# HengWeiBin/CenterFusionDetect3D

Hardware: AMD Instinct MI355X
Metric: frames/sec/GPU CenterFusion forward, 3x448x800 bs=16; 1/2/4/8-GPU scaling (higher is better)
Workload: dtype f32 storage + f32 accumulate; products as split-operand MFMA passes: f16x3 backbone/neck (3 passes), heads' first 3x3 layers fp16 main term + block-scaled FP6 e2m3 cross terms (1.5 passes), heads' 1x1 layers bf16x3; 1 GPU; Centerfusion_Middle (DLA-34 + DCNv2 neck + pc_dep frustum fusion, 7+4 heads) forward + NMS/top-100 decode + 2D->3D postProcess, bs=16/GPU, 3x448x800, 50-200 radar pts/frame, random-init weights; global_batch=16, parallelism=dp1 (batch shard, async all-gather of the final boxes)

## Files before the change

centerfusiondetect3d_amd/_lib.py:

```python
import ctypes as C
import os

_PKG = os.path.dirname(os.path.abspath(__file__))
LIB_PATH = os.path.join(_PKG, "libcfhip.so")

ABI_VERSION = 7
CF_MAX_SRC = 4
CF_MAX_GROUPS = 4
ACT_NONE, ACT_RELU, ACT_SIGMOID_CLAMP, ACT_RAW_AND_SIGDEPTH = 0, 1, 2, 3
LAYOUT_NHWC, LAYOUT_NCHW = 0, 1

_f = C.c_void_p


class ConvArgs(C.Structure):
    _fields_ = [("src", _f * CF_MAX_SRC), ("src_c", C.c_int32 * CF_MAX_SRC), ("n_src", C.c_int32),
                ("B", C.c_int32), ("H", C.c_int32), ("W", C.c_int32), ("Ho", C.c_int32),
                ("Wo", C.c_int32), ("stride", C.c_int32), ("weight", _f), ("slots", _f),
                ("bias", _f), ("K_pad", C.c_int32), ("N", C.c_int32), ("N_pad", C.c_int32),
                ("residual", _f), ("res_stride", C.c_int32), ("out", _f), ("out2", _f),
                ("out_stride", C.c_int32), ("out_layout", C.c_int32), ("act", C.c_int32),
                ("precise", C.c_int32), ("out_scale", C.c_float), ("in_scale", C.c_float)]


# ... 106 lines not shown
class HeadTrainArgs(C.Structure):
    _fields_ = [("x", _f), ("x2", _f), ("x_stride", C.c_int32), ("c_x", C.c_int32), ("x2_stride", C.c_int32),
                ("c_x2", C.c_int32), ("B", C.c_int32), ("h", C.c_int32), ("w", C.c_int32), ("n_hidden", C.c_int32),
                ("hidden", C.c_int32), ("n_out", C.c_int32), ("chunk_px", C.c_int32),
                ("weight", _f * _HT_LAYERS), ("bias", _f * _HT_LAYERS), ("y", _f), ("gy", _f),
                ("gw", _f * _HT_LAYERS), ("gb", _f * _HT_LAYERS), ("workspace", _f), ("workspace_bytes", C.c_size_t)]


CF_TARGETS_MAX_OBJS = 128
CF_TARGETS_F = 20
TGT_HAS_AMODAL, TGT_HAS_ATTRIBUTES, TGT_HAS_VELOCITY, TGT_HAS_ALPHA = 1, 2, 4, 8
TGT_HAS_DEPTH, TGT_HAS_DIMENSION, TGT_HAS_LOCATION, TGT_HAS_YAW = 16, 32, 64, 128
TGT_REP3D, TGT_NORM2D, TGT_WRITE_DEPTH, TGT_WRITE_ROT, TGT_FRUSTUM = 1, 2, 4, 8, 16


class TargetsArgs(C.Structure):
    _fields_ = [("ann", _f), ("iann", _f), ("counts", _f), ("trans", _f), ("calib", _f), ("scale", _f), ("pc_dep", _f),
                ("B", C.c_int32), ("M", C.c_int32), ("C", C.c_int32), ("h", C.c_int32), ("w", C.c_int32),
                ("flags", C.c_int32), ("max_pc_dist", C.c_float),
                ("heat", _f), ("cls", _f), ("mask", _f), ("trunc_mask", _f), ("wh", _f), ("reg", _f), ("amodal_offset", _f),
                ("dimension", _f), ("depth", _f), ("rotbin", _f), ("rotres", _f), ("att", _f), ("att_mask", _f),
                ("velocity", _f), ("pc_hm", _f), ("t_bboxes", _f), ("t_scores", _f), ("t_centers", _f),
                ("t_heat_centers", _f), ("t_bboxes3d", _f), ("t_rotation", _f), ("t_att", _f), ("t_velocity", _f),
                ("workspace", _f), ("workspace_bytes", C.c_size_t)]


_i, _d = C.c_int, C.c_double
SYMBOLS = {
    "cf_conv2d_fused": (_i, [C.POINTER(ConvArgs), _f]),
    "cf_conv2d_f16x3": (_i, [C.POINTER(ConvArgs), _f]),
    "cf_conv3x3_f16x3": (_i, [C.POINTER(ConvArgs), _f]),
    "cf_conv3x3_root_f16x3": (_i, [C.POINTER(ConvArgs), C.POINTER(ConvArgs), C.POINTER(C.c_int32), _f]),
    "cf_conv3x3_proj_f16x3": (_i, [C.POINTER(ConvArgs), C.POINTER(C.c_int32), _f]),
    "cf_conv3x3_f16x3_grouped": (_i, [C.POINTER(C.POINTER(ConvArgs)), C.c_int32, _f]),
    "cf_conv3x3_grouped_form": (_i, [C.POINTER(C.POINTER(ConvArgs)), C.c_int32, C.POINTER(C.c_int32)]),
    "cf_conv3x3_tile_form": (_i, [C.c_int32, C.POINTER(C.POINTER(ConvArgs)), C.c_int32, C.POINTER(C.c_int32), C.POINTER(C.c_int32)]),
    "cf_stem_fused": (_i, [C.POINTER(StemArgs), _f]),
    "cf_stem_fused_early": (_i, [C.POINTER(StemEarlyArgs), _f]),
    "cf_split_bf16": (_i, [_f, _f, C.c_long, _i, _i, _i, _f]),
    "cf_head_fused": (_i, [C.POINTER(HeadFusedArgs), _f]),
    "cf_head_fused_with": (_i, [C.POINTER(HeadFusedArgs), _i, _i, _f]),
    "cf_head_fused_at": (_i, [C.POINTER(HeadFusedArgs), _f, _i, _f]),
    "cf_head_slot_tables": (_i, [_f, _f, _i, _i, _i, _f, _f, _f]),
    "cf_pack_feat_mx": (_i, [_f, _i, _f, C.c_long, _f]),
    "cf_pack_feat_mx_scaled": (_i, [_f, _i, _f, C.c_long, C.c_float, _f]),
    "cf_absmax_f32": (_i, [_f, C.c_long, _i, _i, _f, _f]),
    "cf_dcn_v2_fused": (_i, [C.POINTER(DcnArgs), _f]),
    "cf_dcn_v2_f16x3": (_i, [C.POINTER(DcnArgs), _f]),
    "cf_dcn_v2_workspace_bytes": (C.c_size_t, [_i, _i, _i, _i, _i]),
    "cf_dcn_v2_f16x3_grouped": (_i, [C.POINTER(C.POINTER(DcnArgs)), C.c_int32, _f]),
    "cf_dcn_v2_f16x3_form": (_i, [C.POINTER(C.POINTER(DcnArgs)), C.c_int32, C.POINTER(C.c_int32)]),
    "cf_gemm_tile_form": (_i, [C.c_long, _i, _i, _i, _i, _i, _i, C.POINTER(C.c_int32), C.POINTER(C.c_int32), C.POINTER(C.c_int32)]),
    "cf_dcn_v2_bwd_data": (_i, [C.POINTER(DcnBwdArgs), _f]),
    "cf_dcn_v2_bwd_weight": (_i, [C.POINTER(DcnBwdArgs), _f]),
    "cf_dcn_v2_bwd_workspace_bytes": (C.c_size_t, [_i, _i, _i, _i, _i]),
    "cf_loss_forward": (_i, [C.POINTER(LossArgs), _f]),
    "cf_loss_backward": (_i, [C.POINTER(LossArgs), _f]),
    "cf_loss_workspace_bytes": (C.c_size_t, [_i, _i, _i, _i]),
    "cf_targets_build": (_i, [C.POINTER(TargetsArgs), _f]),
    "cf_targets_workspace_bytes": (C.c_size_t, [_i, _i]),
    "cf_head_train_forward": (_i, [C.POINTER(HeadTrainArgs), _f]),
    "cf_head_backward": (_i, [C.POINTER(HeadTrainArgs), _f]),
    "cf_head_train_workspace_bytes": (C.c_size_t, [_i, _i, _i, _i, _i, _i]),
    "cf_head_bwd_workspace_bytes": (C.c_size_t, [_i, _i, _i, _i, _i, _i]),
    "cf_head_bwd_chunk_px": (_i, [_i, _i, _i, _i]),
    "cf_head_backward_dx": (_i, [C.POINTER(HeadTrainArgs), _f, _i, _f, _i, _f]),
# ... 96 lines not shown
```

centerfusiondetect3d_amd/build.py:

```python
import glob
import os
import shutil
import subprocess
import sys

PKG = os.path.dirname(os.path.abspath(__file__))
ROOT = os.path.dirname(PKG)
CSRC = os.path.join(PKG, "csrc")
OBJ = os.path.join(PKG, "_build")
LIB = os.path.join(PKG, "libcfhip.so")

ARCH = "gfx950"
COMMON = os.environ.get("CF_EXTRA_FLAGS", "").split() + ["-O3", "-std=c++17", "-fPIC", f"-I{os.path.join(ROOT, 'include')}", f"-I{CSRC}"]
SOURCES = [
    ("cf_gemm.hip", []),
    ("cf_gemm_f16.hip", []),
    ("cf_dcn_bwd.hip", []),
    ("cf_neck_bwd.hip", []),
    ("cf_base_bwd.hip", []),
    ("cf_conv3x3_f16.hip", []),
    ("cf_stem.hip", []),
    ("cf_stem_early.hip", []),
    ("cf_heads.hip", []),
    ("cf_heads_bwd.hip", []),
    ("cf_elementwise.hip", []),
    ("cf_topk.hip", ["-ffp-contract=off"]),
    ("cf_frustum.hip", ["-ffp-contract=off"]),
    ("cf_decode.hip", ["-ffp-contract=off"]),
    ("cf_radar.hip", ["-ffp-contract=off"]),
    ("cf_augment.hip", ["-ffp-contract=off"]),
    ("cf_loss.hip", []),
    ("cf_targets.hip", ["-ffp-contract=off"]),
    ("cf_pack.cpp", ["-ffp-contract=off"]),
    ("cf_error.cpp", []),
]


def sources_sha():
    import hashlib
    h = hashlib.sha256()
    files = sorted(glob.glob(os.path.join(CSRC, "*")) + glob.glob(os.path.join(ROOT, "include", "*.h")))
    for f in files:
        h.update(os.path.relpath(f, ROOT).encode() + b"\0")
        h.update(open(f, "rb").read())
    return h.hexdigest()


def _hipcc():
    exe = shutil.which("hipcc") or "/opt/rocm/bin/hipcc"
    if not os.path.exists(exe):
        raise RuntimeError("hipcc not found: cannot build libcfhip.so")
    return exe

# ... 33 lines not shown
```

centerfusiondetect3d_amd/model.py:

```python
import math
import threading
from typing import List

import torch
from torch import nn

from . import _lib, ops, packing
from .packing import Source
from .plan import AT_TIMED, SECONDARY_HEADS, _Plan, feat_operand
from .streams import (_CAPTURE_LOCK, _PROBE_LOG, _PROBE_US, _SIDE_STREAMS,
                      _concurrent, _pick_streams, _side_streams)

CHANNELS = [16, 32, 64, 128, 256, 512]


class _Scope(nn.Module):
    """Empty container: only exists so parameters get the reference's dotted names."""


def _register(root: nn.Module, dotted: str, tensor: torch.Tensor, buffer=False):
    mod = root
    parts = dotted.split(".")
    for p in parts[:-1]:
        if not hasattr(mod, p):
# ... 131 lines not shown
        self.fusionStrategy = config.MODEL.FUSION_STRATEGY if self.isRadarEnabled else None
        if self.fusionStrategy not in (None, "middle", "early"):
            raise NotImplementedError(f"fusion strategy {self.fusionStrategy!r} is outside the hot path")
        self.isEarly = early
        self.isFrustumEnabled = self.isRadarEnabled and bool(config.MODEL.FRUSTUM) and not early
        try:
            config.defrost()
            config.MODEL.PYRAMID_OUT_SIZE = [config.MODEL.OUTPUT_SIZE]
            config.freeze()
        except Exception:
            pass
        for name, tensor, is_buf in _param_spec(config):
            _register(self, name, tensor, is_buf)
        self._packed = None
        self._plans = {}
        self._plan_sets = {}
        self._graphs = {}
        self.max_plan_sets = 4
        self._lock = threading.RLock()
        self.precise = True
        self.conv_f16 = True
        self.lanes = True
        self.lanes_max_frames = 10
        self.streams = 2
        self.trunk_on_caller = True
        self.min_sub_batch = 6
        self.use_graph = False
        self.stem_fused = True
        self.stem_pool = True
        self.conv_patch = True
        self.neck_groups = True
        self.root_fuse = True
        self.root_fuse_children = False
        self.heads_lanes = True
        self.heads_at_peaks = True
        self.peaks_behind_frustum = True
        self.frustum_fused = True
        self.proj_fuse = True
        self.heads_bf16 = True
        self.heads_mx = True
        self._mx_active = False
        self.pack_mx_fused = True
        self.record_spans = False
        self.trunk_spans = []
        self._ranges = None
        self._feat_scale = ops.DEFAULT_IN_SCALE
        self.range_headroom = 8.0
        self._range_checked = False
        self.register_load_state_dict_post_hook(lambda m, _k: m._weights_changed())
        self.freezeBackbone = bool(getattr(config.MODEL, "FREEZE_BACKBONE", False))
        if self.freezeBackbone:
            for name, p in self.named_parameters():
                p.requires_grad_(name.startswith("detectHead_0."))
        self._stale = False
        self._neck_train = False
        self._base_train = False
        self.eval()

    def train(self, mode=True):
        super().train(mode)
        if not mode:
            self._repack_if_stale()
        return self

    def _repack_if_stale(self):
        if getattr(self, "_stale", False):
# ... 869 lines not shown
```

centerfusiondetect3d_amd/ops.py:

```python
import ctypes as C
from typing import Optional, Sequence

import torch

from . import _lib
from ._lib import (ACT_NONE, ACT_RELU, ACT_SIGMOID_CLAMP, ACT_RAW_AND_SIGDEPTH, LAYOUT_NHWC, LAYOUT_NCHW)
from .packing import PackedConv, PackedDcn, MX_ROW as packing_MX_ROW


def _need_cuda(*ts):
    for t in ts:
        if t is not None and not t.is_cuda:
            raise _lib.CfHipError("libcfhip operators need device tensors (no CPU path)")


DEFAULT_IN_SCALE = 16.0
F16_MAX = 65504.0


IN_SCALE_KEEP_MIN = 2.0 ** -6
IN_SCALE_MAX = 2.0 ** 32
F32_MIN_NORMAL = 2.0 ** -126


# ... 152 lines not shown
                       in_scale=None if in_scales is None else in_scales[g])
              for g, (p_, x) in enumerate(zip(pds, xs))]
    _lib.check(_lib.load().cf_dcn_v2_f16x3_grouped(group_ptrs(blocks), G, _lib.stream_ptr()), "cf_dcn_v2_f16x3_grouped")
    return out


def conv3x3_proj_f16x3(pc: PackedConv, t, pooled, act=ACT_RELU, out=None, in_scale=None):
    _need_cuda(t, pooled)
    assert pc.proj_k > 0, "weights packed without a projection"
    B, H, W, _ = t.shape
    if out is None:
        out = torch.empty((B, H, W, pc.n), device=t.device, dtype=torch.float32)
    a = conv_args(pc, [t, pooled], [t.shape[-1], pooled.shape[-1]], B, H, W, out, out.shape[-1], act, None, 0,
                  LAYOUT_NHWC, None, 0, False, in_scale=in_scale)
    ch = (C.c_int32 * 2)(*[int(c) for c in pc.real_cin])
    _lib.check(_lib.load().cf_conv3x3_proj_f16x3(C.byref(a), ch, _lib.stream_ptr()), "cf_conv3x3_proj_f16x3")
    return out


def conv3x3_root_f16x3(pc2: PackedConv, pc_root: PackedConv, t, x1, children=(), act_root=ACT_RELU, x2_out=None,
                       in_scale=None, root_in_scale=None):
    _need_cuda(t, x1, *children)
    B, H, W, _ = t.shape
    x2 = torch.empty((B, H, W, pc2.n), device=t.device, dtype=torch.float32) if x2_out is None else x2_out
    out = torch.empty((B, H, W, pc_root.n), device=t.device, dtype=torch.float32)
    a = conv_args(pc2, [t], [t.shape[-1]], B, H, W, x2, x2.shape[-1], ACT_RELU, x1, x1.shape[-1], LAYOUT_NHWC, None, 0, False,
                  in_scale=in_scale)
    srcs = [x2, x1, *children]
    r = conv_args(pc_root, srcs, [s.shape[-1] for s in srcs], B, H, W, out, out.shape[-1], act_root, None, 0,
                  LAYOUT_NHWC, None, 0, False, in_scale=root_in_scale)
    ch = (C.c_int32 * len(srcs))(*[int(c) for c in pc_root.real_cin])
    _lib.check(_lib.load().cf_conv3x3_root_f16x3(C.byref(a), C.byref(r), ch, _lib.stream_ptr()), "cf_conv3x3_root_f16x3")
    return out, x2


def run_conv(a: _lib.ConvArgs):
    _lib.check(_lib.load().cf_conv2d_fused(C.byref(a), _lib.stream_ptr()), "cf_conv2d_fused")


def conv2d_fused(pc: PackedConv, srcs, B, H, W, act=ACT_NONE, residual=None, layout=LAYOUT_NHWC,
                 out=None, out2=None, precise=True):
    _need_cuda(*srcs, residual)
    Ho = (H + 2 * pc.pad - pc.kh) // pc.stride + 1
    Wo = (W + 2 * pc.pad - pc.kh) // pc.stride + 1
    dev = srcs[0].device
    if out is None:
        shape = (B, Ho, Wo, pc.n) if layout == LAYOUT_NHWC else (B, pc.n, Ho, Wo)
        out = torch.empty(shape, device=dev, dtype=torch.float32)
    if act == ACT_RAW_AND_SIGDEPTH and out2 is None:
        out2 = torch.empty_like(out)
    a = conv_args(pc, srcs, [s.shape[-1] for s in srcs], B, H, W, out, pc.n, act, residual,
                  residual.shape[-1] if residual is not None else 0, layout, out2, 0, precise)
    run_conv(a)
    return (out, out2) if act == ACT_RAW_AND_SIGDEPTH else out


def split_bf16(x, channels=None, cs=None, out=None):
    _need_cuda(x)
    B, H, W, S = x.shape
    Cc = channels or S
    Cs = cs or ((Cc + 7) // 8) * 8
    if out is None:
        out = torch.empty((B, H, W, 2, Cs), device=x.device, dtype=torch.bfloat16)
    _lib.check(_lib.load().cf_split_bf16(x.data_ptr(), out.data_ptr(), B * H * W, Cc, S, Cs,
                                         _lib.stream_ptr()), "cf_split_bf16")
    return out
# ... 1426 lines not shown
```

centerfusiondetect3d_amd/plan.py:

```python
import ctypes as C
import weakref
from typing import Dict, List

import torch

from . import _lib, ops, packing
from .pending import PendingOutputs
from ._lib import (ACT_NONE, ACT_RELU, ACT_SIGMOID_CLAMP, ACT_RAW_AND_SIGDEPTH, LAYOUT_NHWC, LAYOUT_NCHW)
from .streams import _side_streams

SECONDARY_HEADS = ["velocity", "nuscenes_att", "depth2", "rotation2"]
AT_SLOTS = 18
AT_TIMED = ("at.topk", "at.peaks", "at.tables", "at.primary")


def feat_operand(model):
    if not model._heads_bf():
        return None
    return ((packing.MX_ROW,), torch.uint8) if model._mx_active else ((2, 64), torch.bfloat16)


def act_of(h):
    return ACT_SIGMOID_CLAMP if h == "heatmap" else (ACT_RAW_AND_SIGDEPTH if h in ("depth", "depth2") else ACT_NONE)


class _Plan:

    def __init__(self, model: "DLASeg", B, H, W, device, part="all", feat=None, feat_in=None):
        self.B, self.H, self.W, self.device = B, H, W, device
        self.h4, self.w4 = H // 4, W // 4
        self.part = part
        self.lib = _lib.load()
        self.steps = []
        self.lanes = []
        self.lane = 0
        self.n_events = 0
        self.use_lanes = bool(model.lanes) and part != "heads" and \
            B * (H // 4) * (W // 4) <= (model.lanes_max_frames if part == "all" else min(4, model.lanes_max_frames)) * 112 * 200
        self._side = self._events = None
        self.keep = []
        self.bytes = 0
        self.step_index = {}
        self.step_flops = {}
        self.timed = {}
        self.inputs = {}
        self.hidden = set()
        self.debug = {}
        self.in_step = self.stem = self.x4 = self.feat_producer = None
        self.early, self.direct_step, self.chained, self.feat_bf = bool(model.isEarly), None, [], None
        self._pooled = {}
        self._pre = {}
        self.primary, self.radar, self.frustum, self.K = [], False, False, int(model.config.MODEL.K)
# ... 2 lines not shown
        self.peaks_step = self.topk_step = self.frustum_step = None
        self.pc_hm4 = self.pc_hm8 = None
        self.tk_scores = self.tk_inds = self.tk_cls = self.tk_ws = None
        self.pk_ws = self.ev_peaks = None
        self.at, self.at_tails, self.group_flops, self.group_srcs, self._last = None, {}, {}, {}, None
        self.feat, self.feat_in = feat, feat_in
        self._m, self._pk = model, model._packed
        try:
            if part != "heads":
                self._build_trunk()
            if part not in ("trunk", "base", "stem"):
                self._build_heads()
        finally:
            self._m = self._pk = None

    def _buf(self, *shape, dtype=torch.float32):
        t = torch.empty(shape, device=self.device, dtype=dtype)
        self.bytes += t.numel() * t.element_size()
        self.keep.append(t)
        return t

    def _add(self, name, flops, step, *keep):
        self.keep += keep
        self.step_index[name] = len(self.steps)
        if flops is not None:
            self.step_flops[name] = flops
        self.add_step(step)
        return len(self.steps) - 1

    def _slot(self):
        self.add_step(None)
        return len(self.steps) - 1

    def _conv(self, name, srcs, h, w, act=ACT_RELU, residual=None, out=None, out_stride=None):
        m, B, pc = self._m, self.B, self._pk[name]
        ho = (h + 2 * pc.pad - pc.kh) // pc.stride + 1
        wo = (w + 2 * pc.pad - pc.kh) // pc.stride + 1
        if out is None:
            out = self._buf(B, ho, wo, pc.n)
        a = ops.conv_args(pc, srcs, [s.shape[-1] for s in srcs], B, h, w, out, out_stride or pc.n, act, residual,
                          residual.shape[-1] if residual is not None else 0, LAYOUT_NHWC, None, 0, m.precise,
                          in_scale=m._scale(name) if pc.out_scale > 0 else None)
        self.inputs[name] = list(srcs)
        fn = self.lib.cf_conv2d_fused
        if pc.out_scale > 0:
            fn = self.lib.cf_conv3x3_f16x3 if (pc.patch and m.conv_patch) else self.lib.cf_conv2d_f16x3
        self._add(name, 2.0 * B * ho * wo * pc.n * (pc.kh * pc.kh * sum(int(c) for c in pc.real_cin)), (fn, C.byref(a)), a)
        return out

    def _pool(self, x):
        if x.data_ptr() in self._pooled:
            return self._pooled[x.data_ptr()]
        _, h, w, c = x.shape
        o = self._buf(self.B, h // 2, w // 2, c)
        self.add_step((self.lib.cf_maxpool2x2, x.data_ptr(), o.data_ptr(), self.B, h, w, c))
        self._pooled[x.data_ptr()] = o
        return o

    def _block(self, p, x, residual, pooled=None):
        m, B = self._m, self.B
        _, h, w, _ = x.shape
        t = self._conv(p + ".conv1", [x], h, w)
        _, ho, wo, _ = t.shape
        if pooled is None:
            return self._conv(p + ".conv2", [t], ho, wo, residual=residual if residual is not None else x)
        pc = self._pk[p + ".conv2"]
        o = self._buf(B, ho, wo, pc.n)
        a = ops.conv_args(pc, [t, pooled], [t.shape[-1], pooled.shape[-1]], B, ho, wo, o, pc.n, ACT_RELU, None, 0,
                          LAYOUT_NHWC, None, 0, False, in_scale=m._scale(p + ".conv2"))
        self.inputs[p + ".conv2"], self.inputs[p[:-len(".tree1")] + ".project"] = [t], [pooled]
        ch = (C.c_int32 * 2)(*[int(c) for c in pc.real_cin])
        step = (self.lib.cf_conv3x3_proj_f16x3, C.byref(a), ch) if m.conv_patch else (self.lib.cf_conv2d_f16x3, C.byref(a))
        self._add(p + ".conv2+project", 2.0 * B * ho * wo * pc.n * (9 * pc.real_cin[0] + pc.real_cin[1]), step, a, ch)
        return o

    def _tree(self, p, levels, x, stride, level_root, children=None):
        m, B, pk = self._m, self.B, self._pk
        children = [] if children is None else children
        bottom = self._pool(x) if stride > 1 else x
        proj_fused = levels == 1 and getattr(pk[p + ".tree1.conv2"], "proj_k", 0) > 0
        if proj_fused:
            residual = None
        elif (p + ".project") in pk:
            _, h, w, _ = bottom.shape
            residual = self._conv(p + ".project", [bottom], h, w, act=ACT_NONE)
        else:
            residual = bottom
        if level_root:
            children.append(bottom)
        if levels > 1:
            x1 = self._tree(p + ".tree1", levels - 1, x, stride, False)
            children.append(x1)
            return self._tree(p + ".tree2", levels - 1, x1, 1, False, children)
        x1 = self._block(p + ".tree1", x, residual, pooled=bottom if proj_fused else None)
        _, h, w, _ = x1.shape
        pc2, pcr = pk[p + ".tree2.conv2"], pk[p + ".root"]
        if not (m.root_fuse and m.conv_patch and pc2.out_scale > 0 and pcr.out_scale > 0
                and getattr(pc2, "patch", False) and pc2.stride == 1 and (not children or m.root_fuse_children)):
            x2 = self._block(p + ".tree2", x1, None)
            return self._conv(p + ".root", [x2, x1, *children], h, w)
        t = self._conv(p + ".tree2.conv1", [x1], h, w)
        x2, o = self._buf(B, h, w, pc2.n), self._buf(B, h, w, pcr.n)
        a2 = ops.conv_args(pc2, [t], [t.shape[-1]], B, h, w, x2, pc2.n, ACT_RELU, x1, x1.shape[-1],
                           LAYOUT_NHWC, None, 0, False, in_scale=m._scale(p + ".tree2.conv2"))
        rsrcs = [x2, x1, *children]
        ar = ops.conv_args(pcr, rsrcs, [s_.shape[-1] for s_ in rsrcs], B, h, w, o, pcr.n, ACT_RELU, None, 0,
                           LAYOUT_NHWC, None, 0, False, in_scale=m._scale(p + ".root"))
        self.inputs[p + ".tree2.conv2"], self.inputs[p + ".root"] = [t], [x1, *children]
        self.hidden.add(p + ".root")
        rch = (C.c_int32 * len(rsrcs))(*[int(c) for c in pcr.real_cin])
        flops = 2.0 * B * h * w * (pc2.n * 9 * sum(int(c) for c in pc2.real_cin) + pcr.n * sum(int(c) for c in pcr.real_cin))
        self._add(p + ".tree2.conv2+root", flops, (self.lib.cf_conv3x3_root_f16x3, C.byref(a2), C.byref(ar), rch), a2, ar, rch)
        return o

    def _dcn_node(self, p, x, out=None, feat_producer=False):
        m, B = self._m, self.B
        _, h, w, c = x.shape
        om = self._buf(B, h, w, 32)
        self._conv(p + ".conv_offset_mask", [x], h, w, act=ACT_NONE, out=om, out_stride=32)
        pd = self._pk[p]
        o = self._buf(B, h, w, pd.n) if out is None else out
        ws = None
        if pd.out_scale > 0:
            nbytes = self.lib.cf_dcn_v2_workspace_bytes(B, h, w, pd.c, pd.n_pad)
            ws = self._buf(nbytes, dtype=torch.uint8) if nbytes else None
        a = ops.dcn_args(pd, x, om, 32, B, h, w, o, pd.n, ACT_RELU, precise=m.precise, workspace=ws,
                         in_scale=m._scale(p) if pd.out_scale > 0 else None)
        if feat_producer:
            self.feat_producer = a
        self.inputs[p] = [x]
        fn = self.lib.cf_dcn_v2_f16x3 if pd.out_scale > 0 else self.lib.cf_dcn_v2_fused
        self._add(p, 2.0 * B * h * w * pd.n * 9 * pd.c, (fn, C.byref(a)), a)
        return o
# ... 69 lines not shown
                           layers[i - 1].data_ptr(), summed.data_ptr(), self.B, h, w, c, f))
            layers[i] = self._dcn_node(f"{p}.node_{j}", summed, out=final_out if i == endp - 1 else None,
                                       feat_producer=feat and i == endp - 1)

    def _build_trunk(self):
        m, B, H, W, pk = self._m, self.B, self.H, self.W, self._pk
        if self.early and self.part == "all":
            self.direct_step = self._add("pc_hm_direct", 0.0, None)
        if "base.stem" in pk:
            y0, y1 = None, self._buf(B, H // 2, W // 2, 32)
            y1p = self._buf(B, H // 4, W // 4, 32) if m.stem_pool and self.part != "stem" else None
            if y1p is not None:
                self._pooled[y1.data_ptr()] = y1p
            stem_layers = ("base.base_layer", "base.level0", "base.level1")
            kw = dict(shape=(B, 3, H, W), out_pool=y1p, in_scales=[m._scale(n) for n in stem_layers])
            self.stem = ops.stem_early_args(pk["base.stem"], None, None, y1, **kw) if self.early else \
                ops.stem_args(pk["base.stem"], None, y1, **kw)
            self.hidden.update(stem_layers)
            k_base = 16 * 49 * (6 if self.early else 3)
            self.in_step = self._add("base.stem", 2.0 * B * H * W * (k_base + 16 * 144 + 32 * 144 / 4), None, self.stem)
        else:
            self.in_step = self._slot()
            self.x4 = self._buf(B, H, W, 8 if self.early else 4)
            if self.early:
                self.x4.zero_()
            t = self._conv("base.base_layer", [self.x4], H, W)
            y0 = self._conv("base.level0", [t], H, W)
            y1 = self._conv("base.level1", [y0], H, W)
        layers = [y0, y1]
        if self.part == "stem":
            self.levels = [y1]
            return
        for lvl, levels, root in ((2, 1, False), (3, 2, True), (4, 2, True), (5, 1, True)):
            layers.append(self._tree(f"base.level{lvl}", levels, layers[-1], 2, root))
        self.debug = {f"y{i}": t for i, t in enumerate(layers) if t is not None}
        if self.part == "base":
            self.levels = layers[2:]
            return
        out = [layers[-1]]
        n_ida = len(layers) - 2 - 1
        for i in range(n_ida):
            also = [("ida_up.proj_1", layers[-1])] if i == n_ida - 1 and i > 0 else []
            self._ida(f"dla_up.ida_{i}", layers, len(layers) - i - 2, len(layers), also=also)
            out.insert(0, layers[-1])
        for i, t in enumerate(out):
            self.debug[f"up{i}"] = t
        y = out[:3]
        self._ida("ida_up", y, 0, 3, final_out=self.feat, feat=True)
        feat = self.feat = y[-1]
        spec, pr, M4 = feat_operand(m), self.feat_producer, B * self.h4 * self.w4
        if spec is None:
            self.feat_in = feat
            return
        if self.feat_in is None:
            self.feat_in = self._buf(B, self.h4, self.w4, *spec[0], dtype=spec[1])
        if m._mx_active:
            if pr.out_scale > 0 and pr.N == 64 and pr.N_pad == 64 and bool(m.pack_mx_fused):
                pr.out_mx = self.feat_in.data_ptr()
                pr.mx_scale = m._feat_scale
                pr.workspace = None
            else:
                self._add("feat.pack_mx", None, (self.lib.cf_pack_feat_mx_scaled, feat.data_ptr(), 64, self.feat_in.data_ptr(),
                                                 C.c_long(M4), C.c_float(m._feat_scale)))
        elif pr.out_scale > 0 and pr.N == 64:
            pr.out_split_bf16, pr.split_stride = self.feat_in.data_ptr(), 64
            pr.workspace = None
        else:
# ... 387 lines not shown
```

include/cf_hip.h:

```cpp
#ifndef CF_HIP_H
#define CF_HIP_H

#include <stddef.h>
#include <stdint.h>

#ifdef __cplusplus
extern "C" {
#endif

#define CF_ABI_VERSION 7

#define CF_OK 0
#define CF_EINVAL (-22)
#define CF_ELAUNCH (-5)

#define CF_MAX_SRC 4
#define CF_MAX_GROUPS 4

#define CF_ACT_NONE 0
#define CF_ACT_RELU 1
#define CF_ACT_SIGMOID_CLAMP 2
#define CF_ACT_RAW_AND_SIGDEPTH 3

#define CF_LAYOUT_NHWC 0
// ... 29 lines not shown
  int32_t precise;
  float out_scale;
  float in_scale;
} cf_conv_args;
int cf_conv2d_fused(const cf_conv_args* a, void* stream);

typedef struct cf_stem_args {
  const float* x;
  int32_t B, C, H, W;
  const void* w_base;   const float* b_base;   float scale_base;
  const void* w_level0; const float* b_level0; float scale_level0;
  const void* w_level1; const float* b_level1; float scale_level1;
  float* out;
  float* out_pool;
  float in_scale[3];
} cf_stem_args;
int cf_stem_fused(const cf_stem_args* a, void* stream);

typedef struct cf_stem_early_args {
  cf_stem_args stem;
  const float* pc;
  int32_t pc_h, pc_w;
  const void* w_base_radar;
} cf_stem_early_args;
int cf_stem_fused_early(const cf_stem_early_args* a, void* stream);

int cf_conv2d_f16x3(const cf_conv_args* a, void* stream);

int cf_conv3x3_f16x3(const cf_conv_args* a, void* stream);

int cf_conv3x3_root_f16x3(const cf_conv_args* conv, const cf_conv_args* root, const int32_t* root_channels, void* stream);

int cf_conv3x3_proj_f16x3(const cf_conv_args* a, const int32_t* src_channels, void* stream);

int cf_conv3x3_f16x3_grouped(const cf_conv_args* const* groups, int32_t n_groups, void* stream);
int cf_conv3x3_grouped_form(const cf_conv_args* const* groups, int32_t n_groups, int32_t* form);

#define CF_CONV3_ENTRY_PLAIN 0
#define CF_CONV3_ENTRY_ROOT 1
#define CF_CONV3_ENTRY_PROJ 2
#define CF_CONV3_ENTRY_GROUPED 3
#define CF_CONV3_FORM_INTS 23
int cf_conv3x3_tile_form(int32_t entry, const cf_conv_args* const* blocks, int32_t n_blocks, const int32_t* channels, int32_t* form);

typedef struct cf_pack_src {
  int32_t channels;
  int32_t stride;
  int32_t c_base;
} cf_pack_src;
typedef struct cf_pack_bn {
  const float* gamma; const float* beta; const float* mean; const float* var;
  float eps;
} cf_pack_bn;
typedef struct cf_pack_conv_desc {
  const float* weight;
  const float* bias;
  cf_pack_bn bn;
  int32_t cout, kh, kw, stride;
  int32_t pad;
  int32_t dilation;
  const cf_pack_src* src; int32_t n_src;
  const float* proj_weight;
  const float* proj_bias;
  cf_pack_bn proj_bn;
  cf_pack_src proj;
} cf_pack_conv_desc;
// ... 394 lines not shown
```

Measured before the change: 3186 frames/s.

## Add specialised f16x3 GEMM kernel for DLA tree root 1x1 convolutions

Adds a dedicated kernel for the 1x1 root convolutions of the DLA trees. It reads the concatenated multi-source input directly, splits it into hi/lo fp16 in double-buffered LDS, keeps a register ring of weight fragments, and writes bias and ReLU through an LDS-staged epilogue. It is meant to replace the generic f16x3 conv path, with a tile form picked so the grid fits in one round. An optional fused 2x2 max-pool output is also added but is off by default; in exchange the change brings more kernel instantiations and a new dispatch heuristic.

```diff
diff --git a/centerfusiondetect3d_amd/_lib.py b/centerfusiondetect3d_amd/_lib.py
--- a/centerfusiondetect3d_amd/_lib.py
+++ b/centerfusiondetect3d_amd/_lib.py
@@ -162,6 +162,8 @@
     "cf_conv3x3_f16x3": (_i, [C.POINTER(ConvArgs), _f]),
     "cf_conv3x3_root_f16x3": (_i, [C.POINTER(ConvArgs), C.POINTER(ConvArgs), C.POINTER(C.c_int32), _f]),
     "cf_conv3x3_proj_f16x3": (_i, [C.POINTER(ConvArgs), C.POINTER(C.c_int32), _f]),
+    "cf_root1x1_f16x3": (_i, [C.POINTER(ConvArgs), C.POINTER(C.c_int32), _f, _f]),
+    "cf_root1x1_f16x3_form": (_i, [C.POINTER(ConvArgs), C.POINTER(C.c_int32), C.c_int32, C.POINTER(C.c_int32)]),
     "cf_conv3x3_f16x3_grouped": (_i, [C.POINTER(C.POINTER(ConvArgs)), C.c_int32, _f]),
     "cf_conv3x3_grouped_form": (_i, [C.POINTER(C.POINTER(ConvArgs)), C.c_int32, C.POINTER(C.c_int32)]),
     "cf_conv3x3_tile_form": (_i, [C.c_int32, C.POINTER(C.POINTER(ConvArgs)), C.c_int32, C.POINTER(C.c_int32), C.POINTER(C.c_int32)]),
diff --git a/centerfusiondetect3d_amd/build.py b/centerfusiondetect3d_amd/build.py
--- a/centerfusiondetect3d_amd/build.py
+++ b/centerfusiondetect3d_amd/build.py
@@ -19,6 +19,7 @@
     ("cf_neck_bwd.hip", []),
     ("cf_base_bwd.hip", []),
     ("cf_conv3x3_f16.hip", []),
+    ("cf_root_f16.hip", []),
     ("cf_stem.hip", []),
     ("cf_stem_early.hip", []),
     ("cf_heads.hip", []),
diff --git a/centerfusiondetect3d_amd/csrc/cf_root_f16.hip b/centerfusiondetect3d_amd/csrc/cf_root_f16.hip
--- /dev/null
+++ b/centerfusiondetect3d_amd/csrc/cf_root_f16.hip
@@ -0,0 +1,338 @@
+#include <type_traits>
+#include "cf_f16x3.h"
+
+namespace {
+
+struct RootF {
+  const float* src[CF_MAX_SRC];
+  int src_c[CF_MAX_SRC];
+  int c_end[CF_MAX_SRC];
+  const unsigned char* weight;
+  const float* bias;
+  float* out;
+  float* out_pool;
+  int H, W, M, N, n_rt, n_ks, out_stride, act;
+  int tiles_x, tiles_y;
+  int ny;
+  float out_scale, in_scale;
+};
+
+struct RootSrc {
+  const float* p;
+  int sc, c0;
+};
+__device__ __forceinline__ RootSrc root_src(int k, const float* p0, const float* p1, const float* p2, const float* p3, int s0, int s1,
+                                            int s2, int s3, int e0, int e1, int e2) {
+  const bool in0 = k < e0, in1 = k < e1, in2 = k < e2;
+  return {in0 ? p0 : in1 ? p1 : in2 ? p2 : p3, in0 ? s0 : in1 ? s1 : in2 ? s2 : s3, k - (in0 ? 0 : in1 ? e0 : in2 ? e1 : e2)};
+}
+
+template <int WC, int WP, int CT, int KP, int WD, int MINB>
+__global__ __launch_bounds__(256, MINB) void root1x1_f16x3_kernel(RootF p) {
+  static_assert(WC * WP == 4, "4 waves per workgroup");
+  static_assert((KP / 16) % WD == 0, "the weight ring divides a piece");
+  constexpr int RT = 2;
+  constexpr int PXW = 32 * CT;
+  constexpr int PXB = PXW * WP;
+  constexpr int BROW = KP * 2 + 16;
+  constexpr int PLANE = PXB * BROW;
+  constexpr int BUF = 2 * PLANE;
+  constexpr int KSP = KP / 16;
+  constexpr int NT = PXB * KP / 2048;
+  constexpr int NPX = PXB > 64 ? PXB / 64 : 1;
+  constexpr int EROW = RT * 128 + 16;
+  static_assert(NT >= 1 && (PXB & (PXB - 1)) == 0 && KSP % 2 == 0, "tile form");
+  extern __shared__ __attribute__((aligned(16))) unsigned char smem[];
+
+  const int tid = threadIdx.x, lane = tid & 63, wave = __builtin_amdgcn_readfirstlane(tid >> 6);
+  const int li = lane & 31, h = lane >> 5;
+  const int wc = wave / WP, wp = wave % WP;
+  const int lb = cf_xcd_remap(blockIdx.x, gridDim.x);
+  const int tile = lb / p.ny;
+  const int rt0 = ((lb - tile * p.ny) * WC + wc) * RT;
+  const bool w_ok = rt0 < p.n_rt;
+  const bool t2 = p.tiles_x > 0;
+  int m0 = tile * PXB, ty0 = 0, tx0 = 0, img = 0;
+  if (t2) {
+    const int per = p.tiles_x * p.tiles_y;
+    img = tile / per;
+    const int r = tile - img * per, ty = r / p.tiles_x;
+    ty0 = ty * (PXB / 16);
+    tx0 = (r - ty * p.tiles_x) * 16;
+    m0 = img * p.H * p.W;
+  }
+  auto row_of = [&](int slot, bool& ok) {
+    if (t2) {
+      const int y = ty0 + (slot >> 4), x = tx0 + (slot & 15);
+      ok = y < p.H && x < p.W;
+      return m0 + min(y, p.H - 1) * p.W + min(x, p.W - 1);
+    }
+    ok = m0 + slot < p.M;
+    return min(m0 + slot, p.M - 1);
+  };
+
+  int prow[NPX];
+#pragma unroll
+  for (int j = 0; j < NPX; ++j) {
+    bool ok;
+    prow[j] = row_of(((tid >> 2) + 64 * j) & (PXB - 1), ok);
+  }
+  const int n_c32 = p.n_ks >> 1;
+  f32x4 raw[NT][2];
+  auto load_b = [&](int piece) {
+#pragma unroll
+    for (int i = 0; i < NT; ++i) {
+      const int q = (tid >> 2) + 64 * i;
+      const int c32 = min(piece * (KP / 32) + __builtin_amdgcn_readfirstlane(q / PXB), n_c32 - 1);
+      const int k = c32 * 32;
+      const RootSrc s = root_src(k, p.src[0], p.src[1], p.src[2], p.src[3], p.src_c[0], p.src_c[1], p.src_c[2], p.src_c[3],
+                                 p.c_end[0], p.c_end[1], p.c_end[2]);
+      const float* a = s.p + (size_t)prow[NPX > 1 ? (i % NPX) : 0] * s.sc + s.c0 + (tid & 3) * 8;
+      raw[i][0] = *reinterpret_cast<const f32x4*>(a);
+      raw[i][1] = *reinterpret_cast<const f32x4*>(a + 4);
+    }
+  };
+  auto store_b = [&](unsigned char* buf) {
+#pragma unroll
+    for (int i = 0; i < NT; ++i) {
+      const int q = (tid >> 2) + 64 * i;
+      u32x4 hi, lo;
+      split8(raw[i][0], raw[i][1], hi, lo, p.in_scale);
+      unsigned char* o = buf + (q & (PXB - 1)) * BROW + (q / PXB) * 64 + (tid & 3) * 16;
+      *reinterpret_cast<u32x4*>(o) = hi;
+      *reinterpret_cast<u32x4*>(o + PLANE) = lo;
+    }
+  };
+
+  f32x16 accm[RT][CT], accs[RT][CT];
+#pragma unroll
+  for (int a = 0; a < RT; ++a)
+#pragma unroll
+    for (int b = 0; b < CT; ++b)
+#pragma unroll
+      for (int r = 0; r < 16; ++r) {
+        accm[a][b][r] = 0.0f;
+        accs[a][b][r] = 0.0f;
+      }
+
+  f16x8 wh[WD][RT], wl[WD][RT];
+  auto load_w = [&](f16x8 (&dh)[RT], f16x8 (&dl)[RT], int ks) {
+#pragma unroll
+    for (int rt = 0; rt < RT; ++rt) {
+      dh[rt] = *wfrag16(p.weight, w_ok ? rt0 + rt : 0, ks, 0, p.n_ks, lane);
+      dl[rt] = *wfrag16(p.weight, w_ok ? rt0 + rt : 0, ks, 1, p.n_ks, lane);
+    }
+  };
+  auto mma_kstep = [&](const unsigned char* buf, int kk, const f16x8 (&ah)[RT], const f16x8 (&al)[RT]) {
+    f16x8 xh[CT], xl[CT];
+#pragma unroll
+    for (int ct = 0; ct < CT; ++ct) {
+      const unsigned char* row = buf + (wp * PXW + ct * 32 + li) * BROW + kk * 32 + h * 16;
+      xh[ct] = *reinterpret_cast<const f16x8*>(row);
+      xl[ct] = *reinterpret_cast<const f16x8*>(row + PLANE);
+    }
+#pragma unroll
+    for (int rt = 0; rt < RT; ++rt)
+#pragma unroll
+      for (int ct = 0; ct < CT; ++ct) {
+        accs[rt][ct] = __builtin_amdgcn_mfma_f32_32x32x16_f16(al[rt], xh[ct], accs[rt][ct], 0, 0, 0);
+        accs[rt][ct] = __builtin_amdgcn_mfma_f32_32x32x16_f16(ah[rt], xl[ct], accs[rt][ct], 0, 0, 0);
+        accm[rt][ct] = __builtin_amdgcn_mfma_f32_32x32x16_f16(ah[rt], xh[ct], accm[rt][ct], 0, 0, 0);
+      }
+  };
+
+  const int n_pieces = (p.n_ks + KSP - 1) / KSP, last = n_pieces - 1;
+  load_b(0);
+#pragma unroll
+  for (int d = 0; d < WD / 2; ++d) load_w(wh[d], wl[d], min(d, p.n_ks - 1));
+  store_b(smem);
+  load_b(min(1, last));
+#pragma unroll
+  for (int d = WD / 2; d < WD; ++d) load_w(wh[d], wl[d], min(d, p.n_ks - 1));
+  __syncthreads();
+  auto piece = [&](int c, auto full) {
+    const unsigned char* cur = smem + (c & 1) * BUF;
+    unsigned char* nxt = smem + ((c + 1) & 1) * BUF;
+    const int ks0 = c * KSP, nk = p.n_ks - ks0;
+#pragma unroll
+    for (int kk = 0; kk < KSP; ++kk) {
+      if (decltype(full)::value || kk < nk) {
+        mma_kstep(cur, kk, wh[kk % WD], wl[kk % WD]);
+        load_w(wh[kk % WD], wl[kk % WD], min(ks0 + kk + WD, p.n_ks - 1));
+      }
+      if (kk == 0) {
+        store_b(nxt);
+        load_b(min(c + 2, last));
+      }
+    }
+    __syncthreads();
+  };
+  const int n_full = p.n_ks / KSP;
+  for (int c = 0; c < n_full; ++c) piece(c, std::true_type{});
+  if (n_full < n_pieces) piece(n_full, std::false_type{});
+
+  if (w_ok) {
+    constexpr int LPP = RT * 8, PPI = 64 / LPP;
+    unsigned char* eb = smem + wave * 32 * EROW;
+    const int chunk = lane % LPP, psub = lane / LPP;
+    const int n = rt0 * 32 + chunk * 4;
+    const f32x4 bias4 = *reinterpret_cast<const f32x4*>(p.bias + n);
+    const bool relu = p.act == CF_ACT_RELU;
+    auto final_of = [&](int ploc) {
+      f32x4 v = *reinterpret_cast<const f32x4*>(eb + ploc * EROW + chunk * 16) + bias4;
+      if (relu) {
+#pragma unroll
+        for (int e = 0; e < 4; ++e) v[e] = fmaxf(v[e], 0.0f);
+      }
+      return v;
+    };
+#pragma unroll
+    for (int ct = 0; ct < CT; ++ct) {
+      if (ct) cf_wave_lds_sync();
+#pragma unroll
+      for (int rt = 0; rt < RT; ++rt)
+#pragma unroll
+        for (int g = 0; g < 4; ++g) {
+          f32x4 v;
+#pragma unroll
+          for (int e = 0; e < 4; ++e) v[e] = (accm[rt][ct][g * 4 + e] + accs[rt][ct][g * 4 + e]) * p.out_scale;
+          *reinterpret_cast<f32x4*>(eb + li * EROW + (rt * 32 + 8 * g + 4 * h) * 4) = v;
+        }
+      cf_wave_lds_sync();
+#pragma unroll
+      for (int it = 0; it < 32 / PPI; ++it) {
+        const int ploc = it * PPI + psub;
+        bool ok;
+        const size_t m = (size_t)row_of(wp * PXW + ct * 32 + ploc, ok);
+        const f32x4 v = final_of(ploc);
+        if (ok) *reinterpret_cast<f32x4*>(p.out + m * p.out_stride + n) = v;
+      }
+      if (p.out_pool && t2) {
+        const int Hp = p.H >> 1, Wp = p.W >> 1;
+        const int yo = (ty0 >> 1) + wp * CT + ct;
+#pragma unroll
+        for (int it = 0; it < 8 / PPI; ++it) {
+          const int j = it * PPI + psub, xo = (tx0 >> 1) + j;
+          const f32x4 a = final_of(2 * j), b = final_of(2 * j + 1), cc = final_of(16 + 2 * j), d = final_of(17 + 2 * j);
+          f32x4 r;
+#pragma unroll
+          for (int e = 0; e < 4; ++e) r[e] = fmaxf(fmaxf(a[e], b[e]), fmaxf(cc[e], d[e]));
+          if (yo < Hp && xo < Wp)
+            *reinterpret_cast<f32x4*>(p.out_pool + ((size_t)(img * Hp + yo) * Wp + xo) * p.N + n) = r;
+        }
+      }
+    }
+  }
+}
+
+struct RootForm {
+  int WC, WP, CT, KP, WD, MINB;
+  int tiles_x, tiles_y, ny;
+  long grid;
+};
+constexpr long ROOT_ROUND = 256;
+
+RootForm root_pick(int B, int H, int W, int N, bool pool) {
+  RootForm f{};
+  if (N <= 128) { f.WC = 2; f.WP = 2; f.KP = 64; }
+  else { f.WC = 4; f.WP = 1; f.KP = 128; }
+  f.ny = (N + 64 * f.WC - 1) / (64 * f.WC);
+  for (f.CT = 1; f.CT <= 2; ++f.CT) {
+    const int pxb = 32 * f.CT * f.WP, th = pxb / 16;
+    long tiles;
+    if (pool) {
+      f.tiles_x = (W + 15) / 16;
+      f.tiles_y = (H + th - 1) / th;
+      tiles = (long)B * f.tiles_x * f.tiles_y;
+    } else {
+      f.tiles_x = f.tiles_y = 0;
+      tiles = ((long)B * H * W + pxb - 1) / pxb;
+    }
+    f.grid = tiles * f.ny;
+    if (f.grid <= ROOT_ROUND || f.CT == 2) break;
+  }
+  f.MINB = f.CT == 2 && f.grid <= ROOT_ROUND ? 1 : 2;
+  f.WD = f.CT == 2 && f.MINB == 2 ? 2 : f.KP / 16;
+  return f;
+}
+
+template <int WC, int WP, int CT, int KP, int WD, int MINB>
+bool root_launch_if(const RootForm& f, const RootF& k, hipStream_t st) {
+  if (f.WC != WC || f.WP != WP || f.CT != CT || f.KP != KP || f.WD != WD || f.MINB != MINB) return false;
+  constexpr size_t buf = 2 * (size_t)(32 * CT * WP) * (KP * 2 + 16) * 2, epi = 4 * 32 * (2 * 128 + 16);
+  constexpr size_t dyn = buf > epi ? buf : epi;
+  static CfLdsLimit lds_limit;
+  lds_limit.ensure(root1x1_f16x3_kernel<WC, WP, CT, KP, WD, MINB>, dyn, 16384);
+  hipLaunchKernelGGL((root1x1_f16x3_kernel<WC, WP, CT, KP, WD, MINB>), dim3((unsigned)f.grid), dim3(256), dyn, st, k);
+  return true;
+}
+
+int root_impl(const cf_conv_args* a, const int32_t* src_channels, float* out_pool, bool pool, void* stream, int32_t* report) {
+  CF_REQUIRE(a != nullptr && src_channels != nullptr, "cf_root1x1_f16x3: null args");
+  CF_REQUIRE(a->n_src >= 1 && a->n_src <= CF_MAX_SRC, "cf_root1x1_f16x3: n_src=%d", a->n_src);
+  CF_REQUIRE(a->B > 0 && a->H > 0 && a->W > 0 && a->stride == 1 && a->Ho == a->H && a->Wo == a->W,
+             "cf_root1x1_f16x3: 1x1 / stride 1 only (%dx%d -> %dx%d, stride %d)", a->H, a->W, a->Ho, a->Wo, a->stride);
+  CF_REQUIRE(a->weight && a->bias && a->out, "cf_root1x1_f16x3: null buffer");
+  CF_REQUIRE(a->out_layout == CF_LAYOUT_NHWC && a->out_stride >= a->N && a->out_stride % 4 == 0,
+             "cf_root1x1_f16x3: output must be fp32 NHWC with a stride that is a multiple of 4");
+  CF_REQUIRE(!a->residual, "cf_root1x1_f16x3: no residual");
+  CF_REQUIRE(a->act == CF_ACT_NONE || a->act == CF_ACT_RELU, "cf_root1x1_f16x3: act=%d unsupported", a->act);
+  CF_REQUIRE(a->N > 0 && a->N == a->N_pad && a->N % 64 == 0, "cf_root1x1_f16x3: N=%d N_pad=%d (N == N_pad, a multiple of 64)", a->N, a->N_pad);
+  CF_REQUIRE(a->out_scale > 0.0f, "cf_root1x1_f16x3: out_scale must be the 2^-(s+4) the weights were packed with");
+  long k_sum = 0;
+  for (int i = 0; i < a->n_src; ++i) {
+    CF_REQUIRE(a->src[i] && src_channels[i] > 0 && src_channels[i] % 32 == 0 && src_channels[i] == a->src_c[i],
+               "cf_root1x1_f16x3: source %d: %d channels in rows of %d (a multiple of 32, the whole row)", i, src_channels[i], a->src_c[i]);
+    k_sum += src_channels[i];
+  }
+  CF_REQUIRE(a->K_pad > 0 && k_sum == a->K_pad, "cf_root1x1_f16x3: the sources' channels (%ld) are not K_pad=%d (1x1 only)", k_sum, a->K_pad);
+  const long M = (long)a->B * a->H * a->W;
+  CF_REQUIRE(M < (1L << 30), "cf_root1x1_f16x3: tensor too large");
+  CF_REQUIRE(!pool || (a->H >= 2 && a->W >= 2), "cf_root1x1_f16x3: the pooled output needs a map of at least 2x2");
+  RootF k{};
+  int c_end = 0;
+  for (int i = 0; i < CF_MAX_SRC; ++i) {
+    const bool on = i < a->n_src;
+    k.src[i] = on ? a->src[i] : a->src[0];
+    k.src_c[i] = on ? a->src_c[i] : a->src_c[0];
+    if (on) c_end += src_channels[i];
+    k.c_end[i] = c_end;
+  }
+  k.weight = reinterpret_cast<const unsigned char*>(a->weight);
+  k.bias = a->bias;
+  k.out = a->out;
+  k.out_pool = out_pool;
+  k.H = a->H; k.W = a->W; k.M = (int)M; k.N = a->N;
+  k.n_rt = a->N / 32;
+  k.n_ks = a->K_pad / 16;
+  k.out_stride = a->out_stride; k.act = a->act;
+  k.out_scale = a->out_scale;
+  k.in_scale = cf_resolve_in_scale(a->in_scale);
+  CF_REQUIRE(k.in_scale > 0.0f, "cf_root1x1_f16x3: in_scale must be 0 (= 16) or a power of two");
+  const RootForm f = root_pick(a->B, a->H, a->W, a->N, pool);
+  CF_REQUIRE(f.grid > 0 && f.grid < (1L << 31), "cf_root1x1_f16x3: grid of %ld workgroups", f.grid);
+  if (report) {
+    const int32_t v[11] = {f.WC, f.WP, f.CT, f.KP, f.WD, f.MINB, (int32_t)f.grid, f.tiles_x, f.tiles_y, f.ny,
+                           (int32_t)((f.grid + ROOT_ROUND - 1) / ROOT_ROUND)};
+    for (int i = 0; i < 11; ++i) report[i] = v[i];
+    return CF_OK;
+  }
+  k.tiles_x = f.tiles_x; k.tiles_y = f.tiles_y; k.ny = f.ny;
+  hipStream_t st = (hipStream_t)stream;
+  const bool launched = root_launch_if<2, 2, 1, 64, 4, 2>(f, k, st) || root_launch_if<2, 2, 2, 64, 4, 1>(f, k, st) ||
+                        root_launch_if<2, 2, 2, 64, 2, 2>(f, k, st) || root_launch_if<4, 1, 1, 128, 8, 2>(f, k, st) ||
+                        root_launch_if<4, 1, 2, 128, 8, 1>(f, k, st) || root_launch_if<4, 1, 2, 128, 2, 2>(f, k, st);
+  CF_REQUIRE(launched, "cf_root1x1_f16x3: the picked form <%d, %d, %d, %d, %d, %d> is not instantiated", f.WC, f.WP, f.CT, f.KP, f.WD, f.MINB);
+  return cf_check_launch("cf_root1x1_f16x3");
+}
+
+}
+
+extern "C" int cf_root1x1_f16x3(const cf_conv_args* a, const int32_t* src_channels, float* out_pool, void* stream) {
+  return root_impl(a, src_channels, out_pool, out_pool != nullptr, stream, nullptr);
+}
+
+extern "C" int cf_root1x1_f16x3_form(const cf_conv_args* a, const int32_t* src_channels, int32_t pool, int32_t* form) {
+  CF_REQUIRE(form != nullptr, "cf_root1x1_f16x3_form: null output");
+  return root_impl(a, src_channels, nullptr, pool != 0, nullptr, form);
+}
diff --git a/centerfusiondetect3d_amd/model.py b/centerfusiondetect3d_amd/model.py
--- a/centerfusiondetect3d_amd/model.py
+++ b/centerfusiondetect3d_amd/model.py
@@ -187,6 +187,8 @@
         self.neck_groups = True
         self.root_fuse = True
         self.root_fuse_children = False
+        self.root_gemm = True
+        self.root_pool = False
         self.heads_lanes = True
         self.heads_at_peaks = True
         self.peaks_behind_frustum = True
diff --git a/centerfusiondetect3d_amd/ops.py b/centerfusiondetect3d_amd/ops.py
--- a/centerfusiondetect3d_amd/ops.py
+++ b/centerfusiondetect3d_amd/ops.py
@@ -208,6 +208,29 @@
     ch = (C.c_int32 * len(srcs))(*[int(c) for c in pc_root.real_cin])
     _lib.check(_lib.load().cf_conv3x3_root_f16x3(C.byref(a), C.byref(r), ch, _lib.stream_ptr()), "cf_conv3x3_root_f16x3")
     return out, x2
+
+
+def root1x1_f16x3(pc: PackedConv, srcs, B, H, W, act=ACT_RELU, pool=False, out=None, in_scale=None):
+    _need_cuda(*srcs, out)
+    if out is None:
+        out = torch.empty((B, H, W, pc.n), device=srcs[0].device, dtype=torch.float32)
+    pooled = torch.empty((B, H // 2, W // 2, pc.n), device=srcs[0].device, dtype=torch.float32) if pool else None
+    a = conv_args(pc, srcs, [s.shape[-1] for s in srcs], B, H, W, out, out.shape[-1], act, None, 0, LAYOUT_NHWC, None, 0, False,
+                  in_scale=in_scale)
+    ch = (C.c_int32 * len(srcs))(*[int(c) for c in pc.real_cin])
+    _lib.check(_lib.load().cf_root1x1_f16x3(C.byref(a), ch, _lib.ptr(pooled), _lib.stream_ptr()), "cf_root1x1_f16x3")
+    return out, pooled
+
+
+ROOT_FORM_FIELDS = ("WC", "WP", "CT", "KP", "WD", "MINB", "grid", "tiles_x", "tiles_y", "ny", "rounds")
+
+
+def root1x1_form(a: _lib.ConvArgs, channels, pool=False):
+    form = (C.c_int32 * len(ROOT_FORM_FIELDS))()
+    ch = (C.c_int32 * len(channels))(*[int(c) for c in channels])
+    if _lib.load().cf_root1x1_f16x3_form(C.byref(a), ch, int(bool(pool)), form) != 0:
+        return None
+    return dict(zip(ROOT_FORM_FIELDS, form))
 
 
 def run_conv(a: _lib.ConvArgs):
diff --git a/centerfusiondetect3d_amd/plan.py b/centerfusiondetect3d_amd/plan.py
--- a/centerfusiondetect3d_amd/plan.py
+++ b/centerfusiondetect3d_amd/plan.py
@@ -18,6 +18,11 @@
     if not model._heads_bf():
         return None
     return ((packing.MX_ROW,), torch.uint8) if model._mx_active else ((2, 64), torch.bfloat16)
+
+
+def root_gemm_takes(a, pc, pool):
+    form = ops.root1x1_form(a, pc.real_cin, pool) if pc.out_scale > 0 and pc.kh == 1 and len(pc.real_cin) == a.n_src else None
+    return form is not None and form["rounds"] == 1
 
 
 def act_of(h):
@@ -86,7 +91,7 @@
         self.add_step(None)
         return len(self.steps) - 1
 
-    def _conv(self, name, srcs, h, w, act=ACT_RELU, residual=None, out=None, out_stride=None):
+    def _conv(self, name, srcs, h, w, act=ACT_RELU, residual=None, out=None, out_stride=None, pool_out=False):
         m, B, pc = self._m, self.B, self._pk[name]
         ho = (h + 2 * pc.pad - pc.kh) // pc.stride + 1
         wo = (w + 2 * pc.pad - pc.kh) // pc.stride + 1
@@ -99,7 +104,15 @@
         fn = self.lib.cf_conv2d_fused
         if pc.out_scale > 0:
             fn = self.lib.cf_conv3x3_f16x3 if (pc.patch and m.conv_patch) else self.lib.cf_conv2d_f16x3
-        self._add(name, 2.0 * B * ho * wo * pc.n * (pc.kh * pc.kh * sum(int(c) for c in pc.real_cin)), (fn, C.byref(a)), a)
+        step, keep = (fn, C.byref(a)), ()
+        pool_out = pool_out and bool(m.root_pool) and ho >= 2 and wo >= 2
+        if m.root_gemm and name.endswith(".root") and root_gemm_takes(a, pc, pool_out):
+            pooled = self._buf(B, ho // 2, wo // 2, pc.n) if pool_out else None
+            if pooled is not None:
+                self._pooled[out.data_ptr()] = pooled
+            keep = ((C.c_int32 * len(srcs))(*[int(c) for c in pc.real_cin]),)
+            step = (self.lib.cf_root1x1_f16x3, C.byref(a), keep[0], _lib.ptr(pooled))
+        self._add(name, 2.0 * B * ho * wo * pc.n * (pc.kh * pc.kh * sum(int(c) for c in pc.real_cin)), step, a, *keep)
         return out
 
     def _pool(self, x):
@@ -128,7 +141,7 @@
         self._add(p + ".conv2+project", 2.0 * B * ho * wo * pc.n * (9 * pc.real_cin[0] + pc.real_cin[1]), step, a, ch)
         return o
 
-    def _tree(self, p, levels, x, stride, level_root, children=None):
+    def _tree(self, p, levels, x, stride, level_root, children=None, pool_out=False):
         m, B, pk = self._m, self.B, self._pk
         children = [] if children is None else children
         bottom = self._pool(x) if stride > 1 else x
@@ -145,14 +158,14 @@
         if levels > 1:
             x1 = self._tree(p + ".tree1", levels - 1, x, stride, False)
             children.append(x1)
-            return self._tree(p + ".tree2", levels - 1, x1, 1, False, children)
+            return self._tree(p + ".tree2", levels - 1, x1, 1, False, children, pool_out)
         x1 = self._block(p + ".tree1", x, residual, pooled=bottom if proj_fused else None)
         _, h, w, _ = x1.shape
         pc2, pcr = pk[p + ".tree2.conv2"], pk[p + ".root"]
         if not (m.root_fuse and m.conv_patch and pc2.out_scale > 0 and pcr.out_scale > 0
                 and getattr(pc2, "patch", False) and pc2.stride == 1 and (not children or m.root_fuse_children)):
             x2 = self._block(p + ".tree2", x1, None)
-            return self._conv(p + ".root", [x2, x1, *children], h, w)
+            return self._conv(p + ".root", [x2, x1, *children], h, w, pool_out=pool_out)
         t = self._conv(p + ".tree2.conv1", [x1], h, w)
         x2, o = self._buf(B, h, w, pc2.n), self._buf(B, h, w, pcr.n)
         a2 = ops.conv_args(pc2, [t], [t.shape[-1]], B, h, w, x2, pc2.n, ACT_RELU, x1, x1.shape[-1],
@@ -288,7 +301,7 @@
             self.levels = [y1]
             return
         for lvl, levels, root in ((2, 1, False), (3, 2, True), (4, 2, True), (5, 1, True)):
-            layers.append(self._tree(f"base.level{lvl}", levels, layers[-1], 2, root))
+            layers.append(self._tree(f"base.level{lvl}", levels, layers[-1], 2, root, pool_out=lvl < 5))
         self.debug = {f"y{i}": t for i, t in enumerate(layers) if t is not None}
         if self.part == "base":
             self.levels = layers[2:]
diff --git a/include/cf_hip.h b/include/cf_hip.h
--- a/include/cf_hip.h
+++ b/include/cf_hip.h
@@ -85,6 +85,9 @@
 int cf_conv3x3_root_f16x3(const cf_conv_args* conv, const cf_conv_args* root, const int32_t* root_channels, void* stream);
 
 int cf_conv3x3_proj_f16x3(const cf_conv_args* a, const int32_t* src_channels, void* stream);
+
+int cf_root1x1_f16x3(const cf_conv_args* a, const int32_t* src_channels, float* out_pool, void* stream);
+int cf_root1x1_f16x3_form(const cf_conv_args* a, const int32_t* src_channels, int32_t pool, int32_t* form);
 
 int cf_conv3x3_f16x3_grouped(const cf_conv_args* const* groups, int32_t n_groups, void* stream);
 int cf_conv3x3_grouped_form(const cf_conv_args* const* groups, int32_t n_groups, int32_t* form);
```

Result: no change. 3185 frames/s (-0.1%).
